# LUMC/kPAL

Measured on AMD Instinct MI355X. Metric: Gbases/s k-mer counted (k=12, 150bp synthetic), higher is better.
Workload: dtype int64

## Files before the change

kpal_amd/csrc/kpal_ctx.hip:

```cpp
#include "kpal_host.hpp"

static thread_local char g_err[512] = "";

int set_err(int code, const char *fmt, ...)
{
    va_list ap;
    va_start(ap, fmt);
    vsnprintf(g_err, sizeof(g_err), fmt, ap);
    va_end(ap);
    return code;
}

KPAL_API const char *kpal_last_error(void) { return g_err; }
KPAL_API const char *kpal_version(void) { return "kpal_amd 0.4 (gfx950)"; }

int ensure(kpal_ctx *ctx, DevBuf &b, size_t bytes)
{
    if (b.cap >= bytes && b.p) return KPAL_OK;
    if (b.p) {
        HIPCHK(hipStreamSynchronize(ctx->stream));
        HIPCHK(hipFree(b.p));
        b.p = nullptr;
        b.cap = 0;
    }
// ... 19 lines not shown

hipEvent_t prof_event(kpal_ctx *ctx)
{
    if (!ctx->ev_pool.empty()) {
        hipEvent_t e = ctx->ev_pool.back();
        ctx->ev_pool.pop_back();
        return e;
    }
    hipEvent_t e = nullptr;
    if (hipEventCreate(&e) != hipSuccess) return nullptr;
    return e;
}

int prof_collect(kpal_ctx *ctx)
{
    if (ctx->prof_pending.empty()) return KPAL_OK;
    HIPCHK(hipStreamSynchronize(ctx->stream));
    if (ctx->comm_stream) HIPCHK(hipStreamSynchronize(ctx->comm_stream));
    for (auto &r : ctx->prof_pending) {
        float ms = 0.f;
        HIPCHK(hipEventElapsedTime(&ms, r.a, r.b));
        ctx->prof_ms[r.name] += ms;
        ctx->prof_launches[r.name] += 1;
        ctx->ev_pool.push_back(r.a);
        ctx->ev_pool.push_back(r.b);
    }
    ctx->prof_pending.clear();
    return KPAL_OK;
}

KPAL_API int kpal_device_count(int *n)
{
    if (!n) return set_err(KPAL_E_INVALID, "n is NULL");
    int c = 0;
    hipError_t e = hipGetDeviceCount(&c);
    if (e != hipSuccess) {
        *n = 0;
        return set_err(KPAL_E_HIP, "hipGetDeviceCount: %s", hipGetErrorString(e));
    }
    *n = c;
    return KPAL_OK;
}

static int ctx_init(kpal_ctx *ctx, int device)
{
    ctx->device = device;
    hipDeviceProp_t prop;
    HIPCHK(hipGetDeviceProperties(&prop, device));
    ctx->num_cu = prop.multiProcessorCount > 0 ? prop.multiProcessorCount : 256;
    {
        char bus[32] = "", path[128];
        if (hipDeviceGetPCIBusId(bus, (int)sizeof(bus), device) == hipSuccess && bus[0]) {
            for (char *q = bus; *q; ++q) *q = (char)tolower((unsigned char)*q);
            snprintf(path, sizeof(path), "/sys/bus/pci/devices/%s/numa_node", bus);
            if (FILE *f = fopen(path, "r")) {
                int node = -1;
                if (fscanf(f, "%d", &node) == 1 && node >= 0) ctx->numa_node = node;
                fclose(f);
            }
        }
        (void)hipGetLastError();
        HostPool::set_preferred_node(ctx->numa_node);
    }
    HIPCHK(hipStreamCreateWithFlags(&ctx->stream, hipStreamNonBlocking));
    HIPCHK(hipStreamCreateWithFlags(&ctx->copy_stream, hipStreamNonBlocking));
    for (int i = 0; i < 2; ++i) {
        HIPCHK(hipEventCreateWithFlags(&ctx->ev_copied[i], hipEventDisableTiming));
        HIPCHK(hipEventCreateWithFlags(&ctx->ev_done[i], hipEventDisableTiming));
    }
    if (const char *e = getenv("KPAL_BATCH_BYTES")) {
        unsigned long long v = strtoull(e, nullptr, 10);
        if (v >= (1ULL << 20)) {
            ctx->batch_bytes = (size_t)v;
            ctx->batch_bytes_set = true;
        }
    }
    if (const char *e = getenv("KPAL_LEVEL2")) ctx->level2_mode = atoi(e);
    if (const char *e = getenv("KPAL_FASTA_CHUNK")) {
        const unsigned long long v = strtoull(e, nullptr, 10);
        if (v >= 16 && v <= kpal_ctx::kStage) ctx->fa_chunk = (size_t)v;
    }
    if (const char *e = getenv("KPAL_QUAD_STEPS")) ctx->quad_steps_forced = atoi(e);
    if (const char *e = getenv("KPAL_QUAD_STEPS2")) ctx->quad_steps2_forced = atoi(e);
    if (const char *e = getenv("KPAL_QUAD_VERBOSE")) ctx->quad_verbose = atoi(e) != 0;
    if (const char *e = getenv("KPAL_QUAD_REPEAT")) ctx->quad_repeat_forced = atoi(e) != 0 ? 1 : 0;
    if (const char *e = getenv("KPAL_HIST_PACKED")) ctx->quad_hist_unpacked = atoi(e) == 0;
    if (const char *e = getenv("KPAL_DIRECT_SEG")) {
        const long v = atol(e);
        if (v >= 1 && v <= (1 << 20)) {
            ctx->direct_seg = (uint32_t)v;
            ctx->direct_seg_forced = true;
        }
    }
    if (const char *e = getenv("KPAL_SPLIT_ABOVE")) {
        unsigned long long v = strtoull(e, nullptr, 10);
        if (v >= 1024) ctx->split_above = v;
    }
    if (const char *e = getenv("KPAL_QUAD_POOL_MAX")) {
        unsigned long long v = strtoull(e, nullptr, 10);
        if (v >= ((size_t)1 << 20) && v < ((size_t)30 << 30)) ctx->quad_pool_max = (size_t)v;
    }
    return KPAL_OK;
}

KPAL_API void kpal_ctx_destroy(kpal_ctx *ctx);

KPAL_API int kpal_ctx_create(int device, kpal_ctx **out)
{
    if (!out) return set_err(KPAL_E_INVALID, "out is NULL");
    *out = nullptr;
    int n = 0;
    HIPCHK(hipGetDeviceCount(&n));
    if (device < 0 || device >= n) return set_err(KPAL_E_INVALID, "device %d not in 0..%d", device, n - 1);
    HIPCHK(hipSetDevice(device));
    kpal_ctx *ctx = new (std::nothrow) kpal_ctx();
    if (!ctx) return set_err(KPAL_E_NOMEM, "out of host memory");
    const int rc = ctx_init(ctx, device);
    if (rc != KPAL_OK) {
        ctx->device = device;
        kpal_ctx_destroy(ctx);
        return rc;
    }
    *out = ctx;
    return KPAL_OK;
}

KPAL_API int kpal_comm_destroy(kpal_ctx *ctx);

KPAL_API void kpal_ctx_destroy(kpal_ctx *ctx)
{
    if (!ctx) return;
    (void)hipSetDevice(ctx->device);
    (void)hipDeviceSynchronize();
    (void)kpal_comm_destroy(ctx);
    DevBuf *bufs[] = {&ctx->table, &ctx->keys, &ctx->cntmat, &ctx->offs, &ctx->bucket_start, &ctx->slice_start, &ctx->chunk_meta, &ctx->chunk_table, &ctx->chunk_ovf, &ctx->chunk_sorted, &ctx->quad_meta, &ctx->quad_meta2, &ctx->direct_list, &ctx->direct_meta, &ctx->residuals, &ctx->cnt1, &ctx->offs1, &ctx->start1, &ctx->fa_raw[0], &ctx->fa_raw[1], &ctx->fa_flat[0], &ctx->fa_flat[1], &ctx->fa_meta[0], &ctx->fa_meta[1], &ctx->fa_tail, &ctx->fq_raw[0], &ctx->fq_raw[1], &ctx->fq_flat[0], &ctx->fq_flat[1], &ctx->fq_meta, &ctx->fq_pos, &ctx->fq_status, &ctx->rec_raw, &ctx->rec_flat, &ctx->rec_meta, &ctx->rec_starts, &ctx->rec_hdr, &ctx->win_index, &ctx->win_tiles, &ctx->xsend, &ctx->xrecv, &ctx->dstage[0],
                      &ctx->dstage[1], &ctx->scratch[0], &ctx->scratch[1], &ctx->scratch[2], &ctx->scratch[3],
                      &ctx->partials, &ctx->result, &ctx->canon, &ctx->opt_l, &ctx->opt_r, &ctx->opt_levels, &ctx->opt_profiles, &ctx->near_dist, &ctx->near_best};
    for (DevBuf *b : bufs)
        if (b->p) (void)hipFree(b->p);
    if (ctx->fa_nflat_host) (void)hipHostFree(ctx->fa_nflat_host);
    if (ctx->fq_status_host) (void)hipHostFree(ctx->fq_status_host);
    if (ctx->fq_ev) (void)hipEventDestroy(ctx->fq_ev);
    for (void *p : ctx->host_allocs) (void)hipHostFree(p);
    for (int i = 0; i < 2; ++i) {
        if (ctx->pinned[i]) (void)hipHostFree(ctx->pinned[i]);
        if (ctx->ev_copied[i]) (void)hipEventDestroy(ctx->ev_copied[i]);
        if (ctx->ev_done[i]) (void)hipEventDestroy(ctx->ev_done[i]);
    }
    for (auto &r : ctx->prof_pending) {
        (void)hipEventDestroy(r.a);
        (void)hipEventDestroy(r.b);
    }
    for (auto e : ctx->ev_pool) (void)hipEventDestroy(e);
    if (ctx->stream) (void)hipStreamDestroy(ctx->stream);
    if (ctx->copy_stream) (void)hipStreamDestroy(ctx->copy_stream);
    delete ctx;
}

KPAL_API int kpal_sync(kpal_ctx *ctx)
{
    CTX_ENTER(ctx);
    if (ctx->counting) CHK(table_ready(ctx));
    HIPCHK(hipStreamSynchronize(ctx->stream));
    if (ctx->comm_stream) HIPCHK(hipStreamSynchronize(ctx->comm_stream));
    return KPAL_OK;
}
// ... 91 lines not shown
```

kpal_amd/csrc/kpal_host.hpp:

```cpp
#pragma once
#include "../../include/kpal_hip.h"

#include <hip/hip_runtime.h>

#include <algorithm>
#include <cmath>
#include <cstdarg>
#include <cstdio>
#include <cstdlib>
#include <cstring>
#include <string>
#include <thread>
#include <type_traits>
#include <vector>

#include "kpal_device.hpp"
#include "host_pool.hpp"
#include "quad_plan.hpp"
#include "matrix_plan.hpp"
#include "fastq_mask.hpp"
#include "record_scan.hpp"

#define KPAL_API extern "C" __attribute__((visibility("default")))

// ... 8 lines not shown
            return set_err(e_ == hipErrorOutOfMemory ? KPAL_E_NOMEM : KPAL_E_HIP, "%s failed: %s (%s:%d)", \
                           #expr, hipGetErrorString(e_), __FILE__, __LINE__);                      \
    } while (0)

#define CHK(expr)              \
    do {                       \
        int rc_ = (expr);      \
        if (rc_ != KPAL_OK) return rc_; \
    } while (0)


struct DevBuf {
    void *p = nullptr;
    size_t cap = 0;
};

struct ProfRec {
    int name;
    hipEvent_t a, b;
};

struct QuadFinalize {
    bool pending = false;
    const void *stage = nullptr;
    bool fresh = false;
    bool resolved = false;
    Span span = {};
    uint32_t nseg = 0;
    uint32_t seg = 16384;
    uint32_t seg_hist = 16384;

    void arm(const void *stage_, bool fresh_ = false, const Span &span_ = {}, uint32_t nseg_ = 0, uint32_t seg_ = 0, uint32_t seg_hist_ = 0)
    {
        pending = true;
        stage = stage_;
        fresh = fresh_;
        resolved = false;
        if (fresh_) {
            span = span_;
            nseg = nseg_;
            seg = seg_;
            seg_hist = seg_hist_;
        }
    }
    bool needs_resolve() const { return pending && fresh && !resolved; }
    void resolve() { resolved = true; }
    bool take()
    {
        const bool was_fresh = fresh;
        pending = fresh = false;
        return was_fresh;
    }
    void clear() { pending = fresh = false; }
};

struct RecordFileScan {
    RecordScan scan;
    bool fastq = false;
    FqMask mask = {-1, 33};
    uint64_t records = 0;
};

struct kpal_ctx {
    int device = 0;
    hipStream_t stream = nullptr;
    hipStream_t copy_stream = nullptr;
    int num_cu = 256;
    int numa_node = -1;
    int k = 0;
    int strategy = KPAL_STRATEGY_AUTO;
    bool counting = false;
    DevBuf table;
    uint64_t bins = 0;
    size_t batch_bytes = (size_t)1 << 30;
    bool batch_bytes_set = false;
    uint64_t split_above = 0xFFFFFFFFull;
    size_t quad_pool_max = (size_t)30 << 30;
    DevBuf keys, cntmat, offs, bucket_start, slice_start;
    DevBuf chunk_meta, chunk_table, chunk_ovf, chunk_sorted;
    DevBuf quad_meta, quad_meta2;
    uint32_t *quad_error_word = nullptr;
    bool chunk_error_armed = false;
    int quad_steps_forced = 0, quad_steps2_forced = 0;
    bool quad_verbose = false;
    int quad_repeat_forced = -1;
    int plan_strategy = 0, plan_steps1 = 0, plan_steps2 = 0;
    uint64_t stat_fresh_pieces = 0, stat_fresh_reruns = 0, stat_quad_pieces = 0, stat_chunked_pieces = 0, stat_split_pieces = 0, stat_repeat_pieces = 0;
    QuadTileCache tiles;
    QuadFinalize fin;
    bool table_zero_pending = false;
    bool fresh_feed = false;
    DevBuf direct_list, direct_meta;
    uint32_t direct_seg = 16384;
    bool direct_seg_forced = false;
    bool quad_hist_unpacked = false;
    int level2_mode = 2;
    alignas(16) unsigned char chunk_pool_sent[96] = {};
    void *chunk_pool_dev = nullptr;
    uint32_t chunk_meta_y = 0;
    uint32_t *chunk_error_word = nullptr;
    DevBuf residuals, cnt1, offs1, start1;
    DevBuf fa_raw[2], fa_flat[2], fa_meta[2], fa_tail;
    DevBuf rec_raw, rec_flat, rec_meta, rec_starts, rec_hdr;
    std::vector<uint64_t> rec_starts_host, rec_hdr_host;
    uint64_t rec_n = 0, rec_nf = 0;
    RecordFileScan rec_scan;
    DevBuf win_index, win_tiles;
    std::vector<uint64_t> win_first_host, win_tile_host;
    uint64_t win_window = 0, win_step = 0;
    uint64_t *fa_nflat_host = nullptr;
    DevBuf fq_raw[2], fq_flat[2], fq_meta, fq_pos, fq_status;
    unsigned long long *fq_status_host = nullptr;
    hipEvent_t fq_ev = nullptr;
    std::vector<uint8_t> fq_carry;
    uint64_t fq_records = 0;
    FqMask fq_mask = {-1, 33};
    bool fq_open = false;
    std::vector<void *> host_allocs;
    size_t fa_chunk = kStage;
    static constexpr size_t kStage = (size_t)64 << 20;
    static constexpr size_t kStagePad = 64;
    void *pinned[2] = {nullptr, nullptr};
    DevBuf dstage[2];
    hipEvent_t ev_copied[2] = {nullptr, nullptr};
    hipEvent_t ev_done[2] = {nullptr, nullptr};
    bool stage_used[2] = {false, false};
    DevBuf scratch[4];
    DevBuf partials, result;
    DevBuf opt_l, opt_r, opt_levels, opt_profiles;
    DevBuf near_dist, near_best;
    DevBuf canon;
    std::vector<uint32_t> canon_host;
    int canon_k = 0;
    void *comm = nullptr;
    int comm_rank = 0, comm_world = 1;
    hipStream_t comm_stream = nullptr;
    hipEvent_t ev_table_copied = nullptr;
    hipEvent_t ev_side_free[2] = {nullptr, nullptr};
    bool side_used[2] = {false, false};
    DevBuf side[2];
    int side_turn = 0;
    void *merged = nullptr;
    uint64_t merged_bins = 0;
    uint64_t merged_first = 0;
    DevBuf xsend, xrecv;
    bool prof = false;
    std::vector<std::string> prof_names;
    std::vector<double> prof_ms;
    std::vector<uint64_t> prof_launches;
    std::vector<ProfRec> prof_pending;
    std::vector<hipEvent_t> ev_pool;
    uint64_t prof_dropped = 0;
};


int ensure(kpal_ctx *ctx, DevBuf &b, size_t bytes);
int prof_name_id(kpal_ctx *ctx, const char *name);
hipEvent_t prof_event(kpal_ctx *ctx);
int prof_collect(kpal_ctx *ctx);

struct ProfScope {
    kpal_ctx *ctx;
    ProfRec rec;
    bool on;
    ProfScope(kpal_ctx *c, const char *name) : ctx(c), on(c->prof)
    {
// ... 149 lines not shown
```

kpal_amd/csrc/kpal_quads.hip:

```cpp
#include "kpal_host.hpp"

#include "quad_kernels.hpp"

int quad_meta(kpal_ctx *ctx, QuadMeta *out)
{
    CHK(ensure(ctx, ctx->quad_meta, ((size_t)ctx->num_cu + 4 + 2048 + 512) * sizeof(uint32_t)));
    out->nrounds = (uint32_t *)ctx->quad_meta.p;
    out->error = out->nrounds + ctx->num_cu;
    out->load = out->error + 4;
    if (!ctx->quad_error_word) {
        HIPCHK(hipMemsetAsync(out->error, 0, 4 * sizeof(uint32_t), ctx->stream));
        ctx->quad_error_word = out->error;
    }
    return KPAL_OK;
}

int quad_choose_steps(kpal_ctx *ctx, const Span &s, uint32_t *load, int buckets, int slots, const int *candidates, size_t n_candidates,
                      int *steps_out, std::vector<double> *fine)
{
    const int extra = fine ? kQuadFineRows : 0;
    const QuadSampleGrid g = quad_sample_grid((s.nchunks + 63) / 64);
    HIPCHK(hipMemsetAsync(load, 0, (size_t)(buckets + extra + 1) * sizeof(uint32_t), ctx->stream));
    DISPATCH_K_8_16(ctx->k, LAUNCH(ctx, "quad_sample", (quad_sample_kernel<K>), dim3(g.groups), dim3(512), s, g.stride, g.sample_steps, load));
    std::vector<uint32_t> h((size_t)(buckets + extra + 1));
    HIPCHK(hipMemcpyAsync(h.data(), load, h.size() * sizeof(uint32_t), hipMemcpyDeviceToHost, ctx->stream));
    HIPCHK(hipStreamSynchronize(ctx->stream));
    QuadVerdict v = quad_sample_verdict(h.data(), buckets, fine ? h.data() + buckets : nullptr, h[(size_t)(buckets + extra)], g.sampled_steps,
                                        ctx->strategy == KPAL_STRATEGY_AUTO);
    if (ctx->quad_verbose)
        fprintf(stderr, "[kpal quad] sample: %.2f %% of the items are the excess of the 32 fullest rows, %.0f %% of it in three rows\n",
                v.hot_percent, v.top3_percent);
    if (v.use_chunked) return kQuadsUseChunked;
    ctx->tiles.hot_rows = v.hot_rows;
    const QuadWalk w = quad_walk_level1(v.loads, slots, candidates, n_candidates, v.budget);
    if (ctx->quad_verbose)
        for (size_t ci = 0; ci < w.tried; ++ci)
            fprintf(stderr, "[kpal quad] sample: %d steps per wave -> expected backlog %.0f items (fullest row %.1f of %d)\n", candidates[ci],
                    w.backlog[ci], v.loads.back() * kQuadWaves * candidates[ci], slots);
    *steps_out = w.steps;
    if (fine) *fine = std::move(v.fine);
    return KPAL_OK;
}

int launch_partition_quads(kpal_ctx *ctx, const Span &s)
{
    const uint64_t total_steps = (s.nchunks + 63) / 64;
    if (total_steps == 0) return KPAL_OK;
    const int buckets = ctx->k == 12 ? QuadCfg<12>::kBuckets : 512;
    const int slots = ctx->k == 12 ? QuadCfg<12>::kItems : kQuadRowWords / buckets;
    QuadMeta meta;
    CHK(quad_meta(ctx, &meta));
    uint32_t *nrounds = meta.nrounds, *error = meta.error;
    static const int candidates[] = {8, 7, 6, 4, 3, 2, 1};
    constexpr size_t n_candidates = sizeof(candidates) / sizeof(candidates[0]);
    const size_t feed_bytes = (size_t)(s.hi - s.emit_from);
    int steps = quad_forced_steps(ctx->quad_steps_forced, candidates, n_candidates);
    if (!steps && ctx->tiles.hit(feed_bytes, 1)) steps = ctx->tiles.steps1;
    const bool sampled = !steps;
    if (sampled) {
        CHK(quad_choose_steps(ctx, s, meta.load, buckets, slots, candidates, n_candidates, &steps));
        ctx->tiles.store(steps, 0, feed_bytes);
    }
    const QuadTile tile = quad1_tile(steps, sampled, ctx->tiles.hot_rows, ctx->quad_steps_forced, ctx->quad_repeat_forced);
    steps = tile.steps;
    const bool repeat = tile.repeat;
    if (tile.counted) ++ctx->stat_repeat_pieces;
    ctx->plan_strategy = KPAL_STRATEGY_PARTITION_QUADS;
    ctx->plan_steps1 = steps;
    ctx->plan_steps2 = 0;
    const Quad1Geometry geo = quad1_geometry(total_steps, steps, ctx->num_cu);
    if (geo.too_large) return set_err(KPAL_E_INVALID, "quad partition: batch too large");
    if (geo.pool_bytes > ctx->quad_pool_max && s.nchunks > 64) return kSplitBatch;
    const uint32_t G = geo.G;
    const uint64_t tpb = geo.tpb;
    CHK(ensure(ctx, ctx->keys, geo.pool_bytes));
    uint32_t *pool = (uint32_t *)ctx->keys.p;
    const TableOnly table = {(unsigned long long *)ctx->table.p};
    static const bool allow_staged = [] { const char *e = getenv("KPAL_K12_STAGED"); return !e || atoi(e) != 0; }();
    uint32_t *stage = nullptr;
    if (ctx->k == 12 && allow_staged && (double)feed_bytes <= 240.0 * 4.0 * (double)ctx->bins) {
        CHK(ensure(ctx, ctx->residuals, (size_t)ctx->bins * 4 * sizeof(quad2_stage_t)));
        stage = (uint32_t *)ctx->residuals.p;
    }
#define KPAL_QUAD_LAUNCH(S)                                                                                                  \
    do {                                                                                                                     \
        if (repeat)                                                                                                          \
            LAUNCH(ctx, "quad_scatter", (quad_scatter_kernel<K, 16, S, (S == 8 ? 4 : S), TableOnly, (S != 7)>), dim3(G), dim3(1024), s, tpb, pool, (uint32_t)tpb, \
                   nrounds, error, table);                                                                                   \
        else                                                                                                                 \
            LAUNCH(ctx, "quad_scatter", (quad_scatter_kernel<K, 16, S, (S == 8 && K != 12 ? 4 : S), TableOnly, false>), dim3(G), dim3(1024), s, tpb, pool,    \
                   (uint32_t)tpb, nrounds, error, table);                                                                    \
    } while (0)
    DISPATCH_K_8_12(ctx->k, {
        switch (steps) {
        case 8: KPAL_QUAD_LAUNCH(8); break;
        case 7: KPAL_QUAD_LAUNCH(7); break;
        case 4: KPAL_QUAD_LAUNCH(4); break;
        case 3: KPAL_QUAD_LAUNCH(3); break;
        case 2: KPAL_QUAD_LAUNCH(2); break;
        case 1: KPAL_QUAD_LAUNCH(1); break;
        default: KPAL_QUAD_LAUNCH(6); break;
        }
        LAUNCH(ctx, "quad_hist", (quad_hist_kernel<K>), dim3(QuadCfg<K>::kHistBuckets), dim3(1024), (const uint32_t *)pool,
               (const uint32_t *)nrounds, G, (uint32_t)tpb, table, stage);
    });
#undef KPAL_QUAD_LAUNCH
    if (stage) ctx->fin.arm(stage);
    if (ctx->quad_verbose) {
        uint32_t st[2] = {0, 0};
        HIPCHK(hipMemcpyAsync(st, error, sizeof(st), hipMemcpyDeviceToHost, ctx->stream));
        HIPCHK(hipStreamSynchronize(ctx->stream));
        fprintf(stderr, "[kpal quad] k=%d steps/wave/tile=%d tiles=%llu workgroups=%u hot-table entries used so far=%u\n", ctx->k, steps,
                (unsigned long long)geo.tiles, G, st[1]);
    }
    return KPAL_OK;
}
```

kpal_amd/csrc/kpal_quads2.hip:

```cpp
#include "kpal_host.hpp"

#include "quad_kernels.hpp"

#ifndef KPAL_L1_DEPTH8
#define KPAL_L1_DEPTH8 4
#endif

int launch_partition2_quads(kpal_ctx *ctx, const Span &s, bool fresh)
{
    const uint64_t total_steps = (s.nchunks + 63) / 64;
    if (total_steps == 0) return KPAL_OK;
    QuadMeta meta;
    CHK(quad_meta(ctx, &meta));
    uint32_t *nrounds1 = meta.nrounds, *error = meta.error;
    static const int candidates[] = {8, 7, 6, 3};
    const size_t feed_bytes = (size_t)(s.hi - s.emit_from);
    const bool cached = ctx->tiles.hit(feed_bytes, 2);
    std::vector<double> fine;
    int chosen = ctx->tiles.steps1;
    if (!cached) {
        const Quad2Rows rows = quad2_rows(ctx->k);
        CHK(quad_choose_steps(ctx, s, meta.load, (int)(rows.NB1 * rows.REP), (int)rows.S1, candidates, 4, &chosen, &fine));
    }
    const QuadTile tile1 = quad2_tile1(quad_forced_steps(ctx->quad_steps_forced, candidates, 4), chosen, ctx->tiles.hot_rows, ctx->quad_repeat_forced);
    const int steps1 = tile1.steps;
    const bool repeat1 = tile1.repeat;
    if (tile1.counted) ++ctx->stat_repeat_pieces;
    const Quad2Level1 l1 = quad2_level1(ctx->k, total_steps, steps1, ctx->num_cu);
    if (l1.too_large) return set_err(KPAL_E_INVALID, "quad partition: batch too large");
    if (l1.pool1_bytes > ctx->quad_pool_max && s.nchunks > 64) return kSplitBatch;
    int steps2 = cached ? ctx->tiles.steps2 : quad_walk_level2(fine, steps1);
    const int forced2 = quad_forced_steps(ctx->quad_steps2_forced, kQuadCandidates2, sizeof(kQuadCandidates2) / sizeof(kQuadCandidates2[0]));
    const Quad2Level2 l2 = quad2_level2(l1, forced2 ? forced2 : steps2, ctx->num_cu);
    if (l2.too_large) return set_err(KPAL_E_INVALID, "quad partition: batch too large");
    if (!cached) ctx->tiles.store(steps1, steps2, feed_bytes);
    if (forced2) steps2 = forced2;
    ctx->plan_strategy = KPAL_STRATEGY_PARTITION2_QUADS;
    ctx->plan_steps1 = steps1;
    ctx->plan_steps2 = steps2;
    constexpr int kWaves2 = kQuadWaves;
    const uint32_t NB1 = l1.NB1, G1 = l1.G1, G2 = l2.G2, upw = l2.upw, nseg = l2.nseg;
    const uint64_t tpb1 = l1.tpb1, cap1 = l1.cap1, tiles2 = l2.tiles2, cap2 = l2.cap2;
    CHK(ensure(ctx, ctx->residuals, std::max<size_t>(l1.pool1_bytes, (size_t)ctx->bins * 4 * sizeof(quad2_stage_t))));
    CHK(ensure(ctx, ctx->keys, l2.pool2_bytes));
    CHK(ensure(ctx, ctx->quad_meta2, (size_t)NB1 * G2 * sizeof(uint32_t)));
    uint32_t *pool1 = (uint32_t *)ctx->residuals.p;
    uint32_t *stage = pool1;
    uint32_t *pool2 = (uint32_t *)ctx->keys.p;
    uint32_t *nrounds2 = (uint32_t *)ctx->quad_meta2.p;
    uint32_t seg = 0, seg_h = 0;
    TableSink table = {(unsigned long long *)ctx->table.p, nullptr, nullptr, 0u, nullptr};
    TableSink table2 = table, table_h = table;
    if (fresh) {
        seg = (repeat1 && !ctx->direct_seg_forced) ? ctx->direct_seg * 16u : ctx->direct_seg;
        seg_h = ctx->direct_seg_forced ? seg : std::max<uint32_t>(seg, 1u << 22);
        CHK(ensure(ctx, ctx->direct_list, ((size_t)(nseg - 1) * seg + seg_h) * sizeof(unsigned long long)));
        CHK(ensure(ctx, ctx->direct_meta, ((size_t)nseg + 4) * sizeof(uint32_t)));
        unsigned long long *list = (unsigned long long *)ctx->direct_list.p;
        uint32_t *counts = (uint32_t *)ctx->direct_meta.p, *overflow = counts + nseg;
        HIPCHK(hipMemsetAsync(counts, 0, ((size_t)nseg + 4) * sizeof(uint32_t), ctx->stream));
        table = TableSink{nullptr, list, counts, seg, overflow};
        table2 = TableSink{nullptr, list + (size_t)G1 * seg, counts + G1, seg, overflow};
        table_h = TableSink{nullptr, list + (size_t)(nseg - 1) * seg, counts + (nseg - 1), seg_h, overflow};
    }
#define KPAL_QUAD2_LAUNCH(S2)                                                                                                          \
    do {                                                                                                                               \
        if (repeat1)                                                                                                                   \
            LAUNCH(ctx, "quad2_scatter", (quad2_scatter_kernel<K, kWaves2, S2, true>), dim3(G2, NB1), dim3(kWaves2 * 64), (const uint32_t *)pool1, \
                   (const uint32_t *)nrounds1, G1, (uint32_t)cap1, upw, (uint32_t)tiles2, pool2, (uint32_t)cap2, nrounds2, error, table2); \
        else                                                                                                                           \
            LAUNCH(ctx, "quad2_scatter", (quad2_scatter_kernel<K, kWaves2, S2, false>), dim3(G2, NB1), dim3(kWaves2 * 64), (const uint32_t *)pool1, \
                   (const uint32_t *)nrounds1, G1, (uint32_t)cap1, upw, (uint32_t)tiles2, pool2, (uint32_t)cap2, nrounds2, error, table2); \
    } while (0)
#define KPAL_QUAD1_LAUNCH(S, D)                                                                                                        \
    do {                                                                                                                               \
        if (repeat1 && S != 7)                                                                                                         \
            LAUNCH(ctx, "quad_scatter", (quad_scatter_kernel<K, 16, S, D, TableSink, (S != 7)>), dim3(G1), dim3(1024), s, tpb1, pool1, (uint32_t)cap1, nrounds1, error, table); \
        else                                                                                                                           \
            LAUNCH(ctx, "quad_scatter", (quad_scatter_kernel<K, 16, S, D, TableSink, false>), dim3(G1), dim3(1024), s, tpb1, pool1, (uint32_t)cap1, nrounds1, error, table);    \
    } while (0)
    DISPATCH_K_13_16(ctx->k, {
        if (steps1 == 8) KPAL_QUAD1_LAUNCH(8, KPAL_L1_DEPTH8);
        else if (steps1 == 7) KPAL_QUAD1_LAUNCH(7, 7);
        else if (steps1 == 6) KPAL_QUAD1_LAUNCH(6, 6);
        else KPAL_QUAD1_LAUNCH(3, 3);
        switch (steps2) {
        case 8: KPAL_QUAD2_LAUNCH(8); break;
        case 7: KPAL_QUAD2_LAUNCH(7); break;
        case 6: KPAL_QUAD2_LAUNCH(6); break;
        case 4: KPAL_QUAD2_LAUNCH(4); break;
        case 3: KPAL_QUAD2_LAUNCH(3); break;
        default: KPAL_QUAD2_LAUNCH(2); break;
        }

        if (K >= 15 && (uint64_t)G2 * cap2 * 64 < 65536 && !ctx->quad_hist_unpacked)
            LAUNCH(ctx, "quad_hist", (quad_hist_kernel<K, TableSink, true>), dim3(512, NB1), dim3(1024), (const uint32_t *)pool2, (const uint32_t *)nrounds2,
                   G2, (uint32_t)cap2, table_h, stage);
        else
            LAUNCH(ctx, "quad_hist", (quad_hist_kernel<K, TableSink, false>), dim3(512, NB1), dim3(1024), (const uint32_t *)pool2, (const uint32_t *)nrounds2,
                   G2, (uint32_t)cap2, table_h, stage);
    });
#undef KPAL_QUAD2_LAUNCH
    ctx->fin.arm(stage, fresh, s, nseg, seg, seg_h);
    if (fresh) ctx->table_zero_pending = false;
    return KPAL_OK;
}

int table_ready(kpal_ctx *ctx)
{
    if (ctx->table_zero_pending) {
        HIPCHK(hipMemsetAsync(ctx->table.p, 0, ctx->bins * sizeof(int64_t), ctx->stream));
        ctx->table_zero_pending = false;
    }
    return quad2_finalize(ctx, false);
}

// ... 47 lines not shown
```

kpal_amd/csrc/quad_kernels.hpp:

```cpp
#pragma once
#include <type_traits>

#include "kpal_device.hpp"
#include "quad2_index.hpp"
#include "quad_plan.hpp"

namespace kpal {

constexpr int kQuadSpillCap = 2048;
constexpr int kQuadDummyWords = 4;

template <int K>
struct QuadCfg {
    static_assert(K >= 8 && K <= 16, "quads: k = 8..16");
    static constexpr bool kTwoLevel = K >= 13;
    static constexpr bool kStaged = K >= 12;
    static constexpr int kCoarseBits = kTwoLevel ? 2 * K - 22 : 0;
    static constexpr int kCoarse = 1 << kCoarseBits;
    static constexpr int kRep = kTwoLevel ? (kCoarse >= 256 ? 1 : 256 / kCoarse) : 1;
    static constexpr int kBucketBits = kTwoLevel ? 9 : (K == 12 ? 11 : 9);
    static constexpr int kHistBuckets = 1 << kBucketBits;
    static constexpr int kBuckets = kTwoLevel ? kCoarse * kRep : (1 << kBucketBits);
    static constexpr int kLowBits = kTwoLevel ? 13 : 2 * K - kBucketBits;
    static constexpr int kFormBins = 1 << kLowBits;
// ... 919 lines not shown
            ++round;
#pragma unroll 1
            for (int h = 0; h < FI; h += 4) {
#pragma unroll
                for (int i = 0; i < 4; ++i) rec[i] = quad_pack3(rv[threadIdx.x + (uint32_t)(h + i) * THREADS]);
#pragma unroll
                for (int i = 0; i < 4; ++i) store_rec_at(h + i, rec[i]);
            }
        }
    }
    if (threadIdx.x == 0) nrounds2[wg] = min(round, rounds_cap2);
#pragma unroll
    for (int c = 0; c < CARRY; ++c) quad_items_direct<K, 2, TableSinkRef, KM>(carry_item[c] != 0u, carry_row[c], carry_item[c], table, hot, coarse);
    __syncthreads();
    for (int i = threadIdx.x; i < kQuadHotEntries; i += THREADS) {
        const QuadHot h = hot[i];
        if (h.key && h.count) {
            if (h.key >> 63) {
                sink_add(table, (uint64_t)(h.key & 0x7FFFFFFFFFFFFFFFull), (unsigned long long)h.count);
                continue;
            }
            const uint32_t r = (uint32_t)(h.key >> 32), itm = (uint32_t)h.key;
#pragma unroll
            for (int q = 0; q < 4; ++q)
                if ((itm >> (3 - q)) & 1u) sink_add(table, quad_kmer<K, 2>(r, itm, q, coarse), (unsigned long long)h.count);
        }
    }
    if (sink_arg.list) {
        __syncthreads();
        if (threadIdx.x == 0) sink_arg.count[wg_linear] = min(direct_n, sink_arg.cap);
    }
}

template <int K>
__device__ __forceinline__ uint64_t quad_bin_index(uint32_t row, uint32_t coarse, int i, uint32_t local)
{
    using C = QuadCfg<K>;
    const int sh = C::kLowBits - 6 + 2 * i;
    const uint32_t lopart = local & ((1u << sh) - 1u);
    const uint32_t hipart = local >> sh;
    const uint32_t t = C::kScrBits > 0 ? (lopart >> (sh - C::kScrBits)) : 0u;
    const uint32_t b = row ^ C::smask(t);
    if constexpr (C::kTwoLevel)
        return ((uint64_t)hipart << (C::kCoarseBits + 9 + sh)) | ((uint64_t)(coarse ^ C::smask1(t)) << (9 + sh)) | ((uint64_t)b << sh) | lopart;
    else
        return ((uint64_t)hipart << (C::kBucketBits + sh)) | ((uint64_t)b << sh) | lopart;
}

template <int K, typename SINK = TableOnly, bool PACKED = false>
__global__ __launch_bounds__(1024) void quad_hist_kernel(const uint32_t *__restrict__ pool, const uint32_t *__restrict__ nrounds,
                                                         uint32_t G, uint32_t rounds_cap, SINK table,
                                                         uint32_t *__restrict__ stage)
{
    using C = QuadCfg<K>;
    static_assert(!PACKED || C::kTwoLevel, "packed bins are staged, not merged");
    constexpr int L = C::kLowBits, BINS = C::kFormBins, S = C::kTwoLevel ? 64 : C::kSlots;
    constexpr int PLANES = PACKED ? 2 : 4;
    __shared__ __attribute__((aligned(16))) uint32_t hist[PLANES * BINS + 64];
    auto plane_of = [](int i) -> uint32_t { return (uint32_t)(PACKED ? (i & 1) : i) * (uint32_t)BINS; };
    auto shift_of = [](int i) -> int { return PACKED ? 16 * (i >> 1) : 0; };
    constexpr bool PACK3 = C::kTwoLevel;
    constexpr bool SIBLINGS = C::kPairRows || PACK3;
    const uint32_t row = SIBLINGS ? (((blockIdx.x >> 4) << 4) | ((blockIdx.x & 7u) << 1) | ((blockIdx.x >> 3) & 1u)) : blockIdx.x;
    const uint32_t coarse = blockIdx.y;
    const uint32_t row_linear = coarse * (C::kTwoLevel ? 512u : 0u) + row;
    nrounds += (size_t)coarse * G;
    for (int i = threadIdx.x; i < PLANES * BINS + 64; i += blockDim.x) hist[i] = 0;
    __syncthreads();
    const int lane = threadIdx.x & 63, wave = threadIdx.x >> 6;
    auto stage_swizzle = [](int i, uint32_t local) -> uint32_t {
#if defined(KPAL_AB_NO_STAGE_SWIZZLE)
        return local;
#endif
        if constexpr (C::kStaged) {
            if (i == 0) return local ^ (((local >> 8) & 7u) << 3);
            if (i == 1) return local ^ (((local >> 9) & 7u) << 3);
        }
        return local;
    };
    uint32_t plane_base[2] = {2u * (uint32_t)(BINS * 4), 3u * (uint32_t)(BINS * 4)};
    asm volatile("" : "+v"(plane_base[0]), "+v"(plane_base[1]));
    constexpr bool kUnits = !PACKED;
    auto unit_shift = [](int i) -> int { return kUnits ? 3 - i : 0; };
    auto add_item = [&](uint32_t it, auto guard_tag) {
        constexpr bool GUARD = decltype(guard_tag)::value;
#if defined(KPAL_AB_HIST_TWO_ADDS)
        if constexpr (!GUARD && !PACKED) {
#pragma unroll
            for (int i = 0; i < 4; i += 2) {
                const uint32_t counted = __builtin_amdgcn_ubfe(it, 3 - i, 1) & __builtin_amdgcn_ubfe(it, 2 - i, 1);
                if (KPAL_AB_HIST_TWO_ADDS == 2) {
                    const uint32_t local = __builtin_amdgcn_ubfe(it, 8 - 2 * i, L + 2);
                    atomicAdd(&hist[(uint32_t)(i / 2) * (uint32_t)(2 * BINS) + (local >> 1)], counted << (16u * (local & 1u)));
                } else {
                    atomicAdd(&hist[plane_of(i) + stage_swizzle(i, __builtin_amdgcn_ubfe(it, 10 - 2 * i, L))], counted << unit_shift(i));
                }
            }
            return;
        }
#endif
#if !defined(KPAL_AB_HIST_OLD_SPELLING)
        if constexpr (!GUARD && !PACKED) {
            char *base = reinterpret_cast<char *>(hist);
#pragma unroll
            for (int i = 0; i < 4; ++i) {
                uint32_t off = (it >> (8 - 2 * i)) & (((1u << L) - 1u) << 2);
#if !defined(KPAL_AB_NO_STAGE_SWIZZLE)
                if constexpr (C::kStaged) {
                    if (i == 0) off ^= (off >> 5) & 0xE0u;
                    if (i == 1) off ^= (off >> 6) & 0xE0u;
                }
#endif
                if (i >= 2 && BINS * 4 * 2 > 65535) {
                    const uint32_t shifted = it >> (8 - 2 * i);
                    uint32_t addr;
                    asm("v_bitop3_b32 %0, %1, %2, %3 bitop3:0xea" : "=v"(addr) : "v"(shifted), "s"(((1u << L) - 1u) << 2), "v"(plane_base[i - 2]));
                    atomicAdd(reinterpret_cast<uint32_t *>(base + addr), it & (8u >> i));
                } else {
                    atomicAdd(reinterpret_cast<uint32_t *>(base + ((uint32_t)i * (uint32_t)(BINS * 4) | off)), it & (8u >> i));
                }
            }
            return;
        }
#endif
#if !defined(KPAL_AB_HIST_OLD_SPELLING)
        if constexpr (!GUARD && PACKED) {
            char *base = reinterpret_cast<char *>(hist);
#pragma unroll
            for (int i = 0; i < 4; ++i) {
                uint32_t off = (it >> (8 - 2 * i)) & (((1u << L) - 1u) << 2);
#if !defined(KPAL_AB_NO_STAGE_SWIZZLE)
                if (i == 0) off ^= (off >> 5) & 0xE0u;
                if (i == 1) off ^= (off >> 6) & 0xE0u;
#endif
                const uint32_t value = i < 2 ? __builtin_amdgcn_ubfe(it, 3 - i, 1) : ((it << (13 + i)) & 0x10000u);
                atomicAdd(reinterpret_cast<uint32_t *>(base + ((uint32_t)(i & 1) * (uint32_t)(BINS * 4) | off)), value);
            }
            return;
        }
#endif
#pragma unroll
        for (int i = 0; i < 4; ++i) {
            const uint32_t counted = __builtin_amdgcn_ubfe(it, 3 - i, 1);
            const uint32_t local = stage_swizzle(i, __builtin_amdgcn_ubfe(it, 10 - 2 * i, L));
            if constexpr (GUARD) {
                const uint32_t hot = __builtin_amdgcn_readfirstlane(local);
                const bool eq = counted && local == hot;
                const uint32_t same = (uint32_t)__popcll(__builtin_amdgcn_ballot_w64(eq));
                atomicAdd(&hist[eq ? (uint32_t)(PLANES * BINS + lane) : plane_of(i) + local], counted << (shift_of(i) + unit_shift(i)));
                if (same && lane == (__ffsll((long long)__builtin_amdgcn_ballot_w64(true)) - 1)) atomicAdd(&hist[plane_of(i) + hot], same << (shift_of(i) + unit_shift(i)));
            } else {
                atomicAdd(&hist[plane_of(i) + local], counted << (shift_of(i) + unit_shift(i)));
            }
        }
    };
    auto repeats = [&](const uint4 q) -> bool {
#if defined(KPAL_AB_HIST_NO_SKEWCHECK)
        return false;
#endif
        const uint32_t it = C::kItem3 ? (q.x & 0xFFFFFFu) : q.x;
        const uint32_t first = __builtin_amdgcn_readfirstlane(it);
        return first != 0u && __popcll(__builtin_amdgcn_ballot_w64(it == first)) >= 8;
    };
    auto add4 = [&](const uint4 q, const bool skew) {
        if constexpr (C::kItem3) {
            const uint32_t i0 = q.x, i1 = q.y, i2 = q.z, i3 = q.w;
            const uint32_t i4 = __builtin_amdgcn_perm(q.z, __builtin_amdgcn_perm(q.y, q.x, 0x0c0c0703u), 0x0c070100u);
            if (__builtin_expect(skew, 0)) {
                if (i0 & 15u) add_item(i0, std::true_type{});
                if (i1 & 15u) add_item(i1, std::true_type{});
                if (i2 & 15u) add_item(i2, std::true_type{});
                if (i3 & 15u) add_item(i3, std::true_type{});
                if (i4 & 15u) add_item(i4, std::true_type{});
            } else {
                if (i0 & 15u) add_item(i0, std::false_type{});
                if (i1 & 15u) add_item(i1, std::false_type{});
                if (i2 & 15u) add_item(i2, std::false_type{});
                if (i3 & 15u) add_item(i3, std::false_type{});
#if !defined(KPAL_AB_HIST_NO_RIDER)
                if (i4 & 15u) add_item(i4, std::false_type{});
#endif
            }
            return;
        }
        if (__builtin_expect(skew, 0)) {
            if (q.x) add_item(q.x, std::true_type{});
            if (q.y) add_item(q.y, std::true_type{});
            if (q.z) add_item(q.z, std::true_type{});
            if (q.w) add_item(q.w, std::true_type{});
        } else {
            if (q.x) add_item(q.x, std::false_type{});
            if (q.y) add_item(q.y, std::false_type{});
            if (q.z) add_item(q.z, std::false_type{});
            if (q.w) add_item(q.w, std::false_type{});
        }
    };
    const uint32_t parts = G >= 16u ? 1u : 16u / G;
    const uint32_t g_first = G >= 16u ? (uint32_t)wave : (uint32_t)wave % G;
    const uint32_t part = G >= 16u ? 0u : (uint32_t)wave / G;
    for (uint32_t g = g_first; g < G && part < parts; g += 16) {
        const uint32_t *src3 = pool + ((uint64_t)((row_linear >> 1) * G + g) * rounds_cap) * (uint64_t)(2 * kQuadPackedRecordBytes / 4) +
                               (row_linear & 1u) * (uint32_t)(kQuadPackedRecordBytes / 4);
        const uint4 *src = C::kPairRows
                               ? reinterpret_cast<const uint4 *>(pool + ((uint64_t)((row_linear >> 1) * G + g) * rounds_cap) * (2 * S) + (row_linear & 1u) * S)
                               : reinterpret_cast<const uint4 *>(pool + ((uint64_t)(row_linear * G + g) * rounds_cap) * S);
#if !defined(KPAL_QUAD_NO_PRIO)
        if (parts == 1u) {
            switch (g * 4u / G) {
            case 0: __builtin_amdgcn_s_setprio(3); break;
            case 1: __builtin_amdgcn_s_setprio(2); break;
            case 2: __builtin_amdgcn_s_setprio(1); break;
            default: __builtin_amdgcn_s_setprio(0); break;
            }
        }
#endif
#if defined(KPAL_AB_POOL_FILL)
        const uint32_t nvec = nrounds[g] * (uint32_t)(S / 4) / 7u * 6u;
#else
        const uint32_t nvec = nrounds[g] * (uint32_t)(S / 4);
#endif
        if (nvec == 0u) continue;
        auto fetch = [&](uint32_t at) -> uint4 {
            const uint32_t a = min(at, nvec - 1u);
            uint4 r;
            if constexpr (PACK3) {
                const uint32_t *p3 = src3 + (a >> 4) * (uint32_t)(2 * kQuadPackedRecordBytes / 4) + (a & 15u) * 3u;
                const QuadPacked w = *reinterpret_cast<const QuadPacked *>(p3);
                r = quad_unpack3(w.a, w.b, w.c);
            } else {
                r = src[C::kPairRows ? ((a >> 2) * 8u + (a & 3u)) : a];
            }
            const uint32_t keep = at < nvec ? 0xFFFFFFFFu : 0u;
            r.x &= keep;
            r.y &= keep;
            r.z &= keep;
            r.w &= keep;
            return r;
        };
        uint32_t v = part * 256u + lane;
        uint4 q0 = fetch(v), q1 = fetch(v + 64u), q2 = fetch(v + 128u), q3 = fetch(v + 192u);
        while (v < nvec) {
            v += parts * 256u;
            const uint4 n0 = fetch(v), n1 = fetch(v + 64u), n2 = fetch(v + 128u), n3 = fetch(v + 192u);
#if defined(KPAL_AB_HIST_NO_ADD)
            asm volatile("" ::"v"(q0.x ^ q0.y ^ q0.z ^ q0.w ^ q1.x ^ q1.y ^ q1.z ^ q1.w ^ q2.x ^ q2.y ^ q2.z ^ q2.w ^ q3.x ^ q3.y ^ q3.z ^ q3.w));
#else
            const bool skew = repeats(q0);
            add4(q0, skew);
            add4(q1, skew);
            add4(q2, skew);
            add4(q3, skew);
#endif
            q0 = n0;
            q1 = n1;
            q2 = n2;
            q3 = n3;
        }
    }
#if !defined(KPAL_QUAD_NO_PRIO)
    __builtin_amdgcn_s_setprio(3);
#endif
    __syncthreads();
    if (stage) {
        if constexpr (C::kStaged) {
            using Q = Quad2Index<K>;
            quad2_stage_t *dst = reinterpret_cast<quad2_stage_t *>(stage);
            for (int j = threadIdx.x; j < 4 * BINS / 16; j += blockDim.x) {
                const int i = j / (BINS / 16);
                const uint32_t o = ((uint32_t)j % (uint32_t)(BINS / 16)) * 16u;
                uint32_t c[16];
                uint32_t any = 0;
#pragma unroll
                for (int h = 0; h < 2; ++h) {
                    const uint32_t local = Q::bin_of_word(i, o + 8u * (uint32_t)h);
                    const uint32_t phys = stage_swizzle(i, local) & ~7u;
                    const uint4 *src = reinterpret_cast<const uint4 *>(__builtin_assume_aligned(&hist[plane_of(i) + phys], 16));
                    const uint4 a = src[0];
                    const uint4 b = src[1];
                    c[8 * h + 0] = a.x, c[8 * h + 1] = a.y, c[8 * h + 2] = a.z, c[8 * h + 3] = a.w;
                    c[8 * h + 4] = b.x, c[8 * h + 5] = b.y, c[8 * h + 6] = b.z, c[8 * h + 7] = b.w;
                }
                if constexpr (PACKED) {
                    const int sh = shift_of(i);
#pragma unroll
                    for (int e = 0; e < 16; ++e) c[e] = (c[e] >> sh) & 0xFFFFu;
                } else {
                    const int sh = unit_shift(i);
#pragma unroll
                    for (int e = 0; e < 16; ++e) c[e] >>= sh;
                }
#pragma unroll
                for (int e = 0; e < 16; ++e) any |= c[e];
                if (__builtin_expect(any >= kQuad2StageLimit, 0)) {
#pragma unroll
                    for (int e = 0; e < 16; ++e)
                        if (c[e] >= kQuad2StageLimit) {
                            sink_add(table, quad_bin_index<K>(row, coarse, i, Q::bin_of_word(i, o + (uint32_t)(e & 8)) + (uint32_t)(e & 7)), (unsigned long long)c[e]);
                            c[e] = 0;
                        }
                }
                auto pack = [&](int w) { return c[4 * w] | (c[4 * w + 1] << 8) | (c[4 * w + 2] << 16) | (c[4 * w + 3] << 24); };
                *reinterpret_cast<uint4 *>(dst + Q::word_pos(i, coarse, row, o)) = make_uint4(pack(0), pack(1), pack(2), pack(3));
            }
        }
        return;
    }
#if defined(KPAL_AB_HIST_NO_MERGE)
    return;
#endif
    if constexpr (!PACKED) {
#pragma unroll
        for (int i = 0; i < 4; ++i) {
            for (int local = threadIdx.x; local < BINS; local += blockDim.x) {
                const uint32_t c = hist[i * BINS + stage_swizzle(i, (uint32_t)local)] >> unit_shift(i);
                if (c) atomicAdd(&table.table[quad_bin_index<K>(row, coarse, i, (uint32_t)local)], (unsigned long long)c);
            }
        }
    }
}

template <int K, bool BALANCE, bool FRESH>
__global__ __launch_bounds__(1024) void quad2_finalize_kernel(const quad2_stage_t *__restrict__ stage, unsigned long long *__restrict__ table)
{
    using Q = Quad2Index<K>;
    constexpr int RS = Q::kRowStride;
    using acc_t = typename std::conditional<FRESH, uint32_t, unsigned long long>::type;
    static_assert(!FRESH || 8u * (kQuad2StageLimit - 1u) < 0xFFFFFFFFu, "accumulator width");
    __shared__ acc_t acc[128 * RS];
    uint32_t set_id = blockIdx.x;
    if constexpr (BALANCE) {
        constexpr int SB = Q::kSetBits;
        constexpr int LO = 2 * K - 25 > 0 ? 2 * K - 25 : 0;
        constexpr int HI = 10 < SB - 2 ? 10 : SB - 2;
        constexpr int NN = HI - LO + 1;
        if constexpr (NN > 0 && LO > 0) {
            const uint32_t b = blockIdx.x;
            set_id = ((b & ((1u << NN) - 1u)) << LO) | ((b >> NN) & ((1u << LO) - 1u)) | ((b >> (NN + LO)) << (NN + LO));
        }
    }
// ... 117 lines not shown
```

Baseline: 1585.

## Stream histogram pool reads across row groups with byte-offset prefetch

Replaces the per-group fetch loop in the quad histogram kernel with a streaming request scheme. Each wave keeps running byte offsets, and a partial tail batch of one group is filled with the head of the next non-empty group, so the prefetch pipeline stays full across group boundaries and the per-load clamp and mask work drops out. It also lets an environment variable cap the workgroup count used for quad geometry, and moves the staged-mode switch into the context. The risks are more complex indexing, higher register pressure, and possible correctness issues at the boundaries where groups are stitched together.

After: 1609, median of 6. +1.5%, better.

```diff
diff --git a/kpal_amd/csrc/kpal_ctx.hip b/kpal_amd/csrc/kpal_ctx.hip
--- a/kpal_amd/csrc/kpal_ctx.hip
+++ b/kpal_amd/csrc/kpal_ctx.hip
@@ -125,6 +125,8 @@
     }
     if (const char *e = getenv("KPAL_QUAD_STEPS")) ctx->quad_steps_forced = atoi(e);
     if (const char *e = getenv("KPAL_QUAD_STEPS2")) ctx->quad_steps2_forced = atoi(e);
+    if (const char *e = getenv("KPAL_QUAD_WORKGROUPS")) ctx->quad_workgroups_max = atoi(e);
+    if (const char *e = getenv("KPAL_K12_STAGED")) ctx->k12_staged = atoi(e) != 0;
     if (const char *e = getenv("KPAL_QUAD_VERBOSE")) ctx->quad_verbose = atoi(e) != 0;
     if (const char *e = getenv("KPAL_QUAD_REPEAT")) ctx->quad_repeat_forced = atoi(e) != 0 ? 1 : 0;
     if (const char *e = getenv("KPAL_HIST_PACKED")) ctx->quad_hist_unpacked = atoi(e) == 0;
diff --git a/kpal_amd/csrc/kpal_host.hpp b/kpal_amd/csrc/kpal_host.hpp
--- a/kpal_amd/csrc/kpal_host.hpp
+++ b/kpal_amd/csrc/kpal_host.hpp
@@ -114,6 +114,9 @@
     uint32_t *quad_error_word = nullptr;
     bool chunk_error_armed = false;
     int quad_steps_forced = 0, quad_steps2_forced = 0;
+    int quad_workgroups_max = 0;
+    int quad_cus() const { return quad_workgroups_max > 0 && quad_workgroups_max < num_cu ? quad_workgroups_max : num_cu; }
+    bool k12_staged = true;
     bool quad_verbose = false;
     int quad_repeat_forced = -1;
     int plan_strategy = 0, plan_steps1 = 0, plan_steps2 = 0;
diff --git a/kpal_amd/csrc/kpal_quads.hip b/kpal_amd/csrc/kpal_quads.hip
--- a/kpal_amd/csrc/kpal_quads.hip
+++ b/kpal_amd/csrc/kpal_quads.hip
@@ -68,7 +68,7 @@
     ctx->plan_strategy = KPAL_STRATEGY_PARTITION_QUADS;
     ctx->plan_steps1 = steps;
     ctx->plan_steps2 = 0;
-    const Quad1Geometry geo = quad1_geometry(total_steps, steps, ctx->num_cu);
+    const Quad1Geometry geo = quad1_geometry(total_steps, steps, ctx->quad_cus());
     if (geo.too_large) return set_err(KPAL_E_INVALID, "quad partition: batch too large");
     if (geo.pool_bytes > ctx->quad_pool_max && s.nchunks > 64) return kSplitBatch;
     const uint32_t G = geo.G;
@@ -76,9 +76,8 @@
     CHK(ensure(ctx, ctx->keys, geo.pool_bytes));
     uint32_t *pool = (uint32_t *)ctx->keys.p;
     const TableOnly table = {(unsigned long long *)ctx->table.p};
-    static const bool allow_staged = [] { const char *e = getenv("KPAL_K12_STAGED"); return !e || atoi(e) != 0; }();
     uint32_t *stage = nullptr;
-    if (ctx->k == 12 && allow_staged && (double)feed_bytes <= 240.0 * 4.0 * (double)ctx->bins) {
+    if (ctx->k == 12 && ctx->k12_staged && (double)feed_bytes <= 240.0 * 4.0 * (double)ctx->bins) {
         CHK(ensure(ctx, ctx->residuals, (size_t)ctx->bins * 4 * sizeof(quad2_stage_t)));
         stage = (uint32_t *)ctx->residuals.p;
     }
diff --git a/kpal_amd/csrc/kpal_quads2.hip b/kpal_amd/csrc/kpal_quads2.hip
--- a/kpal_amd/csrc/kpal_quads2.hip
+++ b/kpal_amd/csrc/kpal_quads2.hip
@@ -26,12 +26,12 @@
     const int steps1 = tile1.steps;
     const bool repeat1 = tile1.repeat;
     if (tile1.counted) ++ctx->stat_repeat_pieces;
-    const Quad2Level1 l1 = quad2_level1(ctx->k, total_steps, steps1, ctx->num_cu);
+    const Quad2Level1 l1 = quad2_level1(ctx->k, total_steps, steps1, ctx->quad_cus());
     if (l1.too_large) return set_err(KPAL_E_INVALID, "quad partition: batch too large");
     if (l1.pool1_bytes > ctx->quad_pool_max && s.nchunks > 64) return kSplitBatch;
     int steps2 = cached ? ctx->tiles.steps2 : quad_walk_level2(fine, steps1);
     const int forced2 = quad_forced_steps(ctx->quad_steps2_forced, kQuadCandidates2, sizeof(kQuadCandidates2) / sizeof(kQuadCandidates2[0]));
-    const Quad2Level2 l2 = quad2_level2(l1, forced2 ? forced2 : steps2, ctx->num_cu);
+    const Quad2Level2 l2 = quad2_level2(l1, forced2 ? forced2 : steps2, ctx->quad_cus());
     if (l2.too_large) return set_err(KPAL_E_INVALID, "quad partition: batch too large");
     if (!cached) ctx->tiles.store(steps1, steps2, feed_bytes);
     if (forced2) steps2 = forced2;
diff --git a/kpal_amd/csrc/quad_kernels.hpp b/kpal_amd/csrc/quad_kernels.hpp
--- a/kpal_amd/csrc/quad_kernels.hpp
+++ b/kpal_amd/csrc/quad_kernels.hpp
@@ -1025,7 +1025,7 @@
     asm volatile("" : "+v"(plane_base[0]), "+v"(plane_base[1]));
     constexpr bool kUnits = !PACKED;
     auto unit_shift = [](int i) -> int { return kUnits ? 3 - i : 0; };
-    auto add_item = [&](uint32_t it, auto guard_tag) {
+    auto add_item = [&](uint32_t it, auto guard_tag) __attribute__((always_inline)) {
         constexpr bool GUARD = decltype(guard_tag)::value;
 #if defined(KPAL_AB_HIST_TWO_ADDS)
         if constexpr (!GUARD && !PACKED) {
@@ -1105,7 +1105,7 @@
         const uint32_t first = __builtin_amdgcn_readfirstlane(it);
         return first != 0u && __popcll(__builtin_amdgcn_ballot_w64(it == first)) >= 8;
     };
-    auto add4 = [&](const uint4 q, const bool skew) {
+    auto add4 = [&](const uint4 q, const bool skew) __attribute__((always_inline)) {
         if constexpr (C::kItem3) {
             const uint32_t i0 = q.x, i1 = q.y, i2 = q.z, i3 = q.w;
             const uint32_t i4 = __builtin_amdgcn_perm(q.z, __builtin_amdgcn_perm(q.y, q.x, 0x0c0c0703u), 0x0c070100u);
@@ -1138,18 +1138,87 @@
             if (q.w) add_item(q.w, std::false_type{});
         }
     };
+    const uint32_t wave_u = (uint32_t)__builtin_amdgcn_readfirstlane(wave);
     const uint32_t parts = G >= 16u ? 1u : 16u / G;
-    const uint32_t g_first = G >= 16u ? (uint32_t)wave : (uint32_t)wave % G;
-    const uint32_t part = G >= 16u ? 0u : (uint32_t)wave / G;
-    for (uint32_t g = g_first; g < G && part < parts; g += 16) {
-        const uint32_t *src3 = pool + ((uint64_t)((row_linear >> 1) * G + g) * rounds_cap) * (uint64_t)(2 * kQuadPackedRecordBytes / 4) +
-                               (row_linear & 1u) * (uint32_t)(kQuadPackedRecordBytes / 4);
-        const uint4 *src = C::kPairRows
-                               ? reinterpret_cast<const uint4 *>(pool + ((uint64_t)((row_linear >> 1) * G + g) * rounds_cap) * (2 * S) + (row_linear & 1u) * S)
-                               : reinterpret_cast<const uint4 *>(pool + ((uint64_t)(row_linear * G + g) * rounds_cap) * S);
+    const uint32_t g_first = G >= 16u ? wave_u : wave_u % G;
+    const uint32_t part = G >= 16u ? 0u : wave_u / G;
+    constexpr uint32_t PIECE = PACK3 ? 2u * (uint32_t)kQuadPackedRecordBytes : (C::kPairRows ? 2u : 1u) * (uint32_t)(S * 4);
+    constexpr uint32_t BATCH = PACK3 ? 16u * PIECE : (C::kPairRows ? 8192u : 4096u);
+    const char *rowbase = reinterpret_cast<const char *>(pool) +
+                          ((PACK3 || C::kPairRows) ? ((uint64_t)(row_linear >> 1) * G * rounds_cap) * (uint64_t)PIECE + (row_linear & 1u) * (PIECE / 2u)
+                                                   : ((uint64_t)row_linear * G * rounds_cap) * (uint64_t)PIECE);
+    const uint32_t run_bytes = rounds_cap * PIECE;
+    auto vec_off = [](uint32_t a) -> uint32_t {
+        if constexpr (PACK3) return (a >> 4) * PIECE + (a & 15u) * 12u;
+        return C::kPairRows ? (a >> 2) * 128u + (a & 3u) * 16u : a * 16u;
+    };
+    auto run_vectors = [&](uint32_t g) -> uint32_t {
+#if defined(KPAL_AB_POOL_FILL)
+        return nrounds[g] * (uint32_t)(S / 4) / 7u * 6u;
+#else
+        return nrounds[g] * (uint32_t)(S / 4);
+#endif
+    };
+    auto load = [&](uint32_t o) -> uint4 {
+        if constexpr (PACK3) {
+            const QuadPacked w = *reinterpret_cast<const QuadPacked *>(rowbase + o);
+            return quad_unpack3(w.a, w.b, w.c);
+        } else {
+            return *reinterpret_cast<const uint4 *>(rowbase + o);
+        }
+    };
+    uint32_t nA = 0, pa = 0, gn = part < parts ? g_first : G;
+    uint32_t off[4] = {0u, 0u, 0u, 0u};
+    auto request = [&](uint4 &n0, uint4 &n1, uint4 &n2, uint4 &n3, uint32_t &ok) __attribute__((always_inline)) -> int {
+        const bool whole = pa + 256u <= nA;
+        uint32_t ra = 0, nB = 0, gB = 0;
+        if (!whole) {
+            ra = nA > pa ? nA - pa : 0u;
+#if defined(KPAL_AB_HIST_NO_RIDE)
+            if (ra == 0u)
+#endif
+            while (gn < G) {
+                nB = run_vectors(gn);
+                if (nB) break;
+                gn += 16u;
+            }
+            gB = gn;
+#if defined(KPAL_AB_HIST_NO_RIDE)
+            if (ra == 0u)
+#endif
+            gn += 16u;
+            const uint32_t offB = gB * run_bytes;
+            ok = 0;
+#pragma unroll
+            for (int j = 0; j < 4; ++j) {
+                const uint32_t s = (uint32_t)lane + 64u * (uint32_t)j;
+                const uint32_t b = part * 256u + s - ra;
+                const bool in_a = s < ra, in_b = !in_a && b < nB;
+                off[j] = in_a ? off[j] : (in_b ? offB + vec_off(b) : 0u);
+                ok |= (in_a || in_b ? 1u : 0u) << j;
+            }
+        }
+        n0 = load(off[0]);
+        n1 = load(off[1]);
+        n2 = load(off[2]);
+        n3 = load(off[3]);
+        if (whole) {
+            pa += parts * 256u;
+#pragma unroll
+            for (int j = 0; j < 4; ++j) off[j] += parts * BATCH;
+            return 1;
+        }
+        if (nB == 0u) {
+            nA = pa = 0;
+            return ra ? 2 : 0;
+        }
+        nA = nB;
+        pa = part * 256u + parts * 256u - ra;
+#pragma unroll
+        for (int j = 0; j < 4; ++j) off[j] = gB * run_bytes + vec_off(pa + (uint32_t)lane + 64u * (uint32_t)j);
 #if !defined(KPAL_QUAD_NO_PRIO)
         if (parts == 1u) {
-            switch (g * 4u / G) {
+            switch (gB * 4u / G) {
             case 0: __builtin_amdgcn_s_setprio(3); break;
             case 1: __builtin_amdgcn_s_setprio(2); break;
             case 2: __builtin_amdgcn_s_setprio(1); break;
@@ -1157,34 +1226,23 @@
             }
         }
 #endif
-#if defined(KPAL_AB_POOL_FILL)
-        const uint32_t nvec = nrounds[g] * (uint32_t)(S / 4) / 7u * 6u;
-#else
-        const uint32_t nvec = nrounds[g] * (uint32_t)(S / 4);
-#endif
-        if (nvec == 0u) continue;
-        auto fetch = [&](uint32_t at) -> uint4 {
-            const uint32_t a = min(at, nvec - 1u);
-            uint4 r;
-            if constexpr (PACK3) {
-                const uint32_t *p3 = src3 + (a >> 4) * (uint32_t)(2 * kQuadPackedRecordBytes / 4) + (a & 15u) * 3u;
-                const QuadPacked w = *reinterpret_cast<const QuadPacked *>(p3);
-                r = quad_unpack3(w.a, w.b, w.c);
-            } else {
-                r = src[C::kPairRows ? ((a >> 2) * 8u + (a & 3u)) : a];
-            }
-            const uint32_t keep = at < nvec ? 0xFFFFFFFFu : 0u;
-            r.x &= keep;
-            r.y &= keep;
-            r.z &= keep;
-            r.w &= keep;
-            return r;
-        };
-        uint32_t v = part * 256u + lane;
-        uint4 q0 = fetch(v), q1 = fetch(v + 64u), q2 = fetch(v + 128u), q3 = fetch(v + 192u);
-        while (v < nvec) {
-            v += parts * 256u;
-            const uint4 n0 = fetch(v), n1 = fetch(v + 64u), n2 = fetch(v + 128u), n3 = fetch(v + 192u);
+        return 2;
+    };
+    {
+        uint4 q0, q1, q2, q3;
+        uint32_t q_ok = 0;
+        int kind = request(q0, q1, q2, q3, q_ok);
+        while (kind) {
+            uint4 n0, n1, n2, n3;
+            uint32_t n_ok = 0;
+            const int n_kind = request(n0, n1, n2, n3, n_ok);
+            if (kind == 2) {
+                const uint32_t k0 = 0u - (q_ok & 1u), k1 = 0u - ((q_ok >> 1) & 1u), k2 = 0u - ((q_ok >> 2) & 1u), k3 = 0u - ((q_ok >> 3) & 1u);
+                q0.x &= k0, q0.y &= k0, q0.z &= k0, q0.w &= k0;
+                q1.x &= k1, q1.y &= k1, q1.z &= k1, q1.w &= k1;
+                q2.x &= k2, q2.y &= k2, q2.z &= k2, q2.w &= k2;
+                q3.x &= k3, q3.y &= k3, q3.z &= k3, q3.w &= k3;
+            }
 #if defined(KPAL_AB_HIST_NO_ADD)
             asm volatile("" ::"v"(q0.x ^ q0.y ^ q0.z ^ q0.w ^ q1.x ^ q1.y ^ q1.z ^ q1.w ^ q2.x ^ q2.y ^ q2.z ^ q2.w ^ q3.x ^ q3.y ^ q3.z ^ q3.w));
 #else
@@ -1198,6 +1256,8 @@
             q1 = n1;
             q2 = n2;
             q3 = n3;
+            q_ok = n_ok;
+            kind = n_kind;
         }
     }
 #if !defined(KPAL_QUAD_NO_PRIO)
```
